# cchao0116/EasyDGL

Measured on AMD Instinct MI355X. Metric: sequences/sec (fwd+bwd+Adam) B=512 L=100 d=128 |I|=20K, higher is better.
Workload: dtype bf16

## Files before the change

easydgl_amd/csrc/k_tail.hip:

```cpp
#include "edgl_common.h"

#ifdef EDGL_PHASE_TIMING
__device__ unsigned long long g_phase_cycles[16];
#endif
#if defined(EDGL_PHASE_TIMING) && defined(EDGL_PHASE_BWD)
#define PHB_DECL PH_DECL
#define PHB_MARK(i) PH_MARK(i)
#define PHB_FLUSH() PH_FLUSH(0)
#else
#define PHB_DECL
#define PHB_MARK(i)
#define PHB_FLUSH()
#endif

namespace {

constexpr int MAXRT = 7;

struct TailP {
    const bf16* att; const bf16* xin; int ld_x;
    const bf16 *WoT, *WiT, *WoutT, *WtT;
    const float *bo, *bi, *bout, *bt, *g1, *b1, *g2, *b2, *g3, *b3;
    int B, T, C;
    float rate; const uint64_t* rng; uint32_t sid1, sid2;
    const int64_t* mpos; int M; int head; const int32_t* hmap;
    bf16 *ao, *a1, *pre_f, *f, *o, *y, *pre_t, *so, *hrows;
    float *st1, *st2, *st3;
    int dhp, dht;
};

template <int CT>
struct TailGeom {
    static constexpr int C = 16 * CT, NW = CT, NTHR = 64 * CT, LD = C + 8, CV = C / 8;
    static constexpr int LDF = C + 4;
    static constexpr size_t BUF = (size_t)MAXRT * 16 * LD * sizeof(bf16);
    static_assert((size_t)MAXRT * 16 * LDF * sizeof(float) <= 2 * BUF, "f32 staging image exceeds two buffers");
    static constexpr size_t SMEM = 4 * BUF + 64 * sizeof(float);
    static constexpr size_t SMEM_BWD = SMEM + (size_t)(MAXRT * 16 + 512) * sizeof(int);
    static constexpr int PAR_BO = 0, PAR_BOUT = 1, PAR_G1 = 2, PAR_B1 = 3, PAR_G2 = 4, PAR_B2 = 5, PAR_G3 = 6, PAR_B3 = 7, PAR_BT = 8, PAR_BI = 9;
    static constexpr size_t SMEM_FWD = SMEM + (size_t)11 * C * sizeof(float);
};

template <int CT>
struct RowImage {
    using G = TailGeom<CT>;
    static constexpr int NV = MAXRT * 16 * G::CV, NI = (NV + G::NTHR - 1) / G::NTHR;
    static_assert(NI * G::NTHR - NV < G::NTHR && NV >= G::NTHR, "last round: at most one repeat per thread");
    uint4 d[NI];
    static __device__ __forceinline__ int vec(int i) {
        const int v = threadIdx.x + i * G::NTHR;
        return v < NV ? v : v - (NI * G::NTHR - NV);
    }
    __device__ __forceinline__ void load(const bf16* src, long ld, int T) {
// ... 332 lines not shown
    {
        float mean, rstd;
        joint_moments<CT>(z, nrt, T, lane, red, mean, rstd, cpad);
        if (threadIdx.x == 0) { p.st3[2 * b] = mean; p.st3[2 * b + 1] = rstd; }
        const float4 v_g = *reinterpret_cast<const float4*>(par + G::PAR_G3 * C + nl), v_b = *reinterpret_cast<const float4*>(par + G::PAR_B3 * C + nl);
        const float gv[4] = {v_g.x, v_g.y, v_g.z, v_g.w}, ev[4] = {v_b.x, v_b.y, v_b.z, v_b.w};
#pragma unroll
        for (int rt = 0; rt < MAXRT; ++rt)
            if (rt < nrt) {
                float v[4];
#pragma unroll
                for (int r = 0; r < 4; ++r) v[r] = (z[rt][r] - mean) * rstd * gv[r] + ev[r];
                st_bf4(bufB + (rt * 16 + l15) * LD + nl, v);
            }
    }
    lds_barrier();
    if ((int)threadIdx.x < p.M * G::CV && gat_dst >= 0)
        *reinterpret_cast<uint4*>(p.hrows + gat_dst * C + (threadIdx.x % G::CV) * 8) =
            *reinterpret_cast<const uint4*>(bufB + gat_t * LD + (threadIdx.x % G::CV) * 8);
    for (int v = threadIdx.x + G::NTHR; v < p.M * G::CV; v += G::NTHR) {
        const int j = v / G::CV, cv = v % G::CV;
        const long src = (long)b * p.M + j;
        const int t = (int)p.mpos[src];
        const long dst = p.hmap ? (long)p.hmap[src] : src;
        if (dst >= 0) *reinterpret_cast<uint4*>(p.hrows + dst * C + cv * 8) = *reinterpret_cast<const uint4*>(bufB + t * LD + cv * 8);
    }
#if defined(EDGL_PHASE_TIMING) && !defined(EDGL_PHASE_BWD)
    PH_MARK(0);
    if ((threadIdx.x & 63) == 0) atomicAdd(&g_phase_cycles[8], ph_acc[0]);
#endif
}

struct TailBwdP {
    const bf16 *xin; int ld_x;
    const bf16 *ao, *a1, *pre_f, *o, *pre_t, *so;
    const float *st1, *st2, *st3;
    const bf16 *Wo, *Wi, *Wout, *Wt;
    const float *g1, *g2, *g3;
    int B, T, C;
    float rate; const uint64_t* rng; uint32_t sid1, sid2;
    int head;
    const bf16* d_rows; const int64_t* mpos; int M; const int32_t* rowmap;
    const bf16* d_y_in;
    bf16 *d_pre_t, *d_o, *d_pre_f, *d_ao, *d_res1, *d_att;
    float *part1, *part2, *part3;
    int dhp, dht;
};

template <int CT, int NKB>
__device__ __forceinline__ void tile_dx(const WFrags<NKB>& wf, const bf16* Gs, int nrt, int lane, f32x4 (&acc)[MAXRT]) {
    tile_gemm<CT, NKB>(wf, Gs, nrt, lane, acc);
}

template <int CT>
__device__ __forceinline__ void ln_bwd_regs(const float (&z)[MAXRT][4], const float (&dy)[MAXRT][4], float mean, float rstd,
                                            const float (&gv)[4], int nrt, int T, int lane, int nl, float* red, float* part_b,
                                            float (&dz)[MAXRT][4], const ChanPad& cp) {
    const int l15 = lane & 15;
    const float n = (float)T * cp.ctrue;
    float s1 = 0.f, s2 = 0.f, dga[4] = {0.f, 0.f, 0.f, 0.f}, dbe[4] = {0.f, 0.f, 0.f, 0.f};
#pragma unroll
    for (int rt = 0; rt < MAXRT; ++rt)
        if (rt < nrt && rt * 16 + l15 < T) {
#pragma unroll
            for (int r = 0; r < 4; ++r) {
                const float xh = (z[rt][r] - mean) * rstd, gg = dy[rt][r] * gv[r];
                s1 += gg; s2 += gg * xh; dga[r] += dy[rt][r] * xh; dbe[r] += dy[rt][r];
            }
        }
    const float m1 = block_sum_lds(s1, red) / n;
    const float m2 = block_sum_lds(s2, red) / n;
#pragma unroll
    for (int r = 0; r < 4; ++r) {
#pragma unroll
        for (int o = 1; o < 16; o <<= 1) { dga[r] += __shfl_xor(dga[r], o, 64); dbe[r] += __shfl_xor(dbe[r], o, 64); }
    }
    if (l15 == 0) {
#pragma unroll
        for (int r = 0; r < 4; ++r) { part_b[nl + r] = dbe[r]; part_b[16 * CT + nl + r] = dga[r]; }
    }
#pragma unroll
    for (int rt = 0; rt < MAXRT; ++rt)
#pragma unroll
        for (int r = 0; r < 4; ++r) {
            const float xh = (z[rt][r] - mean) * rstd;
            dz[rt][r] = cp.rm[r] * (rstd * (dy[rt][r] * gv[r] - m1 - xh * m2));
        }
}

template <int CT, int NRT>
__global__ __launch_bounds__(64 * CT) void tail_bwd_kernel(TailBwdP p) {
    using G = TailGeom<CT>;
    constexpr int C = G::C, LD = G::LD, NKB = C / 32;
    extern __shared__ __attribute__((aligned(16))) char smem[];
    bf16* bufA = reinterpret_cast<bf16*>(smem);
    bf16* bufS = reinterpret_cast<bf16*>(smem + G::BUF);
    bf16* bufB = reinterpret_cast<bf16*>(smem + 2 * G::BUF);
    bf16* bufC = reinterpret_cast<bf16*>(smem + 3 * G::BUF);
    float* red = reinterpret_cast<float*>(smem + 4 * G::BUF);
    int* rowmap = reinterpret_cast<int*>(red + 64);
    int* nextj = rowmap + MAXRT * 16;
    int* mpos_s = nextj + 256;
    const int b = blockIdx.x, T = p.T, nrt = NRT ? NRT : (T + 15) / 16;
    const int lane = threadIdx.x & 63, wave = threadIdx.x >> 6, g4 = (lane >> 4) * 4, l15 = lane & 15;
    const int n0 = wave * 16, nl = n0 + g4;
    const long row0 = (long)b * T;
    const ChanPad cpad = chan_pad<CT>(nl, p.dhp, p.dht);
    float z[MAXRT][4], dy[MAXRT][4], dz[MAXRT][4];
    WFrags<NKB> wf = p.head ? load_wfrags<NKB>(p.Wt + (long)n0 * C, C, lane) : load_wfrags<NKB>(p.Wout + (long)n0 * C, C, lane);
    PHB_DECL
    RowImage<CT> im_o, im_a;

    if (p.head) {
        const bool staged = p.M <= MAXRT * 16;
        constexpr int NG = RowImage<CT>::NI;
        int gsrc[NG];
        if (staged && p.rowmap) {
#pragma unroll
            for (int i = 0; i < NG; ++i) gsrc[i] = p.rowmap[(long)b * p.M + min(RowImage<CT>::vec(i) / G::CV, p.M - 1)];
        } else {
#pragma unroll
            for (int i = 0; i < NG; ++i) gsrc[i] = b * p.M + min(RowImage<CT>::vec(i) / G::CV, p.M - 1);
        }
        const int my_pos = (int)p.mpos[(long)b * p.M + min((int)threadIdx.x, p.M - 1)];
        RowImage<CT> im_so, im_dg;
        im_so.load(p.so + row0 * C, C, T);
        im_dg.load(p.pre_t + row0 * C, C, T);
        if (staged) {
            uint4 g[NG];
#pragma unroll
            for (int i = 0; i < NG; ++i)
                g[i] = *reinterpret_cast<const uint4*>(p.d_rows + (long)max(gsrc[i], 0) * C + (RowImage<CT>::vec(i) % G::CV) * 8);
            im_so.store(bufB, T);
            im_dg.store(bufA, T);
#pragma unroll
            for (int i = 0; i < NG; ++i) {
                const int v = RowImage<CT>::vec(i), j = v / G::CV, cv = v % G::CV;
                if (j < p.M) *reinterpret_cast<uint4*>(bufC + j * LD + cv * 8) = gsrc[i] >= 0 ? g[i] : make_uint4(0, 0, 0, 0);
            }
        } else {
// ... 199 lines not shown
#pragma unroll
    for (int rt = 0; rt < MAXRT; ++rt)
        if (rt < nrt) {
            const int row = rt * 16 + l15;
            float v[4], w[4];
#pragma unroll
            for (int r = 0; r < 4; ++r) {
                w[r] = dz[rt][r];
                v[r] = dz[rt][r];
            }
            drop_apply4(dk1, (uint64_t)((row0 + min(row, T - 1)) * C + nl), v);
            st_bf4(bufC + row * LD + nl, v);
            st_bf4(bufS + row * LD + nl, w);
        }
    lds_barrier();
    copy_out<CT>(p.d_ao + row0 * C, C, bufC, T);
    copy_out<CT>(p.d_res1 + row0 * C, C, bufS, T);
    PHB_MARK(6);
    {
        f32x4 acc[MAXRT];
#pragma unroll
        for (int rt = 0; rt < MAXRT; ++rt) acc[rt] = f32x4{0.f, 0.f, 0.f, 0.f};
        tile_dx<CT, NKB>(wf, bufC, nrt, lane, acc);
#pragma unroll
        for (int rt = 0; rt < MAXRT; ++rt)
            if (rt < nrt) {
                const float v[4] = {acc[rt][0], acc[rt][1], acc[rt][2], acc[rt][3]};
                st_bf4(bufA + (rt * 16 + l15) * LD + nl, v);
            }
    }
    lds_barrier();
    copy_out<CT>(p.d_att + row0 * C, C, bufA, T);
    PHB_MARK(7);
    PHB_FLUSH();
}

namespace t2 {
constexpr int C = 128, NTHR = 512, NKB = 4, TMAX = 101;
constexpr int IMG = TMAX * 256;
constexpr int OFF_RED = 3 * IMG, OFF_PAR = OFF_RED + 256;
constexpr int PAR_BOUT = 0, PAR_G2 = 1, PAR_B2 = 2, PAR_G3 = 3, PAR_B3 = 4, PAR_BI = 5, PAR_BT = 7, NPAR = 8;
constexpr int SMEM_FWD = OFF_PAR + NPAR * C * 4;
static_assert(SMEM_FWD == 81920, "two workgroups per CU");
constexpr int OFF_ROWMAP = OFF_RED + 256, OFF_NEXTJ = OFF_ROWMAP + MAXRT * 16 * 4, OFF_MPOS = OFF_NEXTJ + 256 * 4;
constexpr int SMEM_BWD = OFF_MPOS + 256 * 4;
static_assert(SMEM_BWD <= 81920, "two workgroups per CU");

struct Lane {
    int lane, wave, q, l15, nl;
    int frag[NKB];
    int quad;
    int squad;
};
__device__ __forceinline__ Lane make_lane() {
    Lane L;
    L.lane = threadIdx.x & 63; L.wave = threadIdx.x >> 6; L.q = L.lane >> 4; L.l15 = L.lane & 15; L.nl = L.wave * 16 + L.q * 4;
#pragma unroll
    for (int kb = 0; kb < NKB; ++kb) L.frag[kb] = L.l15 * 256 + (((kb * 4 + L.q) ^ L.l15) << 4);
    L.quad = L.l15 * 256 + (((L.wave * 2 + (L.q >> 1)) ^ L.l15) << 4) + ((L.q & 1) << 3);
    L.squad = L.l15 * 512 + (((L.wave * 4 + L.q) ^ L.l15) << 4);
    return L;
}
__device__ __forceinline__ int vec_off(int row, int cv) { return row * 256 + ((cv ^ (row & 15)) << 4); }

template <int NRT>
__device__ __forceinline__ void gemm(const WFrags<NKB>& wf, const char* img, const Lane& L, f32x4 (&acc)[MAXRT]) {
#pragma unroll
    for (int rt = 0; rt < NRT; ++rt) {
#pragma unroll
        for (int kb = 0; kb < NKB; ++kb)
            acc[rt] = mma_kblock(wf.w[kb], *reinterpret_cast<const Vec16<bf16>*>(img + L.frag[kb] + rt * 4096), acc[rt]);
        __builtin_amdgcn_sched_barrier(0);
    }
}
template <int NRT>
__device__ __forceinline__ void zero_acc(f32x4 (&acc)[MAXRT]) {
#pragma unroll
    for (int rt = 0; rt < MAXRT; ++rt) acc[rt] = f32x4{0.f, 0.f, 0.f, 0.f};
}
__device__ __forceinline__ void copy_in2(char* d0, const bf16* s0, long ld0, char* d1, const bf16* s1, long ld1, int T) {
    uint4 a[4], b[4];
    const int nv = T * 16;
#pragma unroll
    for (int i = 0; i < 4; ++i) {
        const int v = min((int)threadIdx.x + i * NTHR, nv - 1), row = v >> 4, cv = v & 15;
        a[i] = *reinterpret_cast<const uint4*>(s0 + (long)row * ld0 + cv * 8);
        b[i] = *reinterpret_cast<const uint4*>(s1 + (long)row * ld1 + cv * 8);
    }
#pragma unroll
    for (int i = 0; i < 4; ++i) {
        const int v = min((int)threadIdx.x + i * NTHR, nv - 1), row = v >> 4, cv = v & 15;
        *reinterpret_cast<uint4*>(d0 + vec_off(row, cv)) = a[i];
        *reinterpret_cast<uint4*>(d1 + vec_off(row, cv)) = b[i];
    }
}
__device__ __forceinline__ void copy_out(bf16* dst, long ld, const char* img, int T) {
    const int nv = T * 16;
#pragma unroll
    for (int i = 0; i < 4; ++i) {
        const int v = threadIdx.x + i * NTHR, row = v >> 4, cv = v & 15;
        if (v < nv) *reinterpret_cast<uint4*>(dst + (long)row * ld + cv * 8) = *reinterpret_cast<const uint4*>(img + vec_off(row, cv));
    }
}
template <int NRT>
__device__ __forceinline__ void stage_acc(char* stg, const f32x4 (&acc)[MAXRT], const Lane& L, int T) {
#pragma unroll
    for (int rt = 0; rt < NRT; ++rt)
        if (rt * 16 + L.l15 < T)
            *reinterpret_cast<float4*>(stg + L.squad + rt * 8192) = make_float4(acc[rt][0], acc[rt][1], acc[rt][2], acc[rt][3]);
}
template <bool SYNC>
__device__ __forceinline__ void gelu_pass(const char* stg, const float* bias_g, bf16* dact_g, bf16* act_g, long ldg, char* act_img, int T) {
    const int cv = threadIdx.x & 15, rsub = threadIdx.x >> 4;
    const float4 b0 = *reinterpret_cast<const float4*>(bias_g + cv * 8), b1 = *reinterpret_cast<const float4*>(bias_g + cv * 8 + 4);
    const int s0 = rsub * 512 + (((2 * cv) ^ (rsub & 15)) << 4);
// ... 148 lines not shown
    if (p.head) touch_regs(wf);
    copy_out(p.o + row0 * C, C, Q, T);
    {
        float mean, rstd;
        joint_moments<8>(z, NRT, T, L.lane, red, mean, rstd, cpad);
        if (threadIdx.x == 0) { p.st2[2 * b] = mean; p.st2[2 * b + 1] = rstd; }
        const float4 v_g = *reinterpret_cast<const float4*>(par + PAR_G2 * C + nl), v_b = *reinterpret_cast<const float4*>(par + PAR_B2 * C + nl);
        const float gv[4] = {v_g.x, v_g.y, v_g.z, v_g.w}, ev[4] = {v_b.x, v_b.y, v_b.z, v_b.w};
#pragma unroll
        for (int rt = 0; rt < NRT; ++rt) {
            float v[4];
#pragma unroll
            for (int r = 0; r < 4; ++r) v[r] = (z[rt][r] - mean) * rstd * gv[r] + ev[r];
            if (rt * 16 + l15 < T) st_bf4(reinterpret_cast<bf16*>(R + L.quad + rt * 4096), v);
        }
    }
    lds_barrier();
    copy_out(p.y + row0 * C, C, R, T);
    if (!p.head) return;
    zero_acc<NRT>(acc);
    gemm<NRT>(wf, R, L, acc);
    stage_acc<NRT>(P, acc, L, T);
    lds_barrier();
    gelu_pass<false>(P, par + PAR_BT * C, p.pre_t + row0 * C, p.so + row0 * C, C, R, T);
    lds_barrier();
#pragma unroll
    for (int rt = 0; rt < NRT; ++rt) ld_bf4(reinterpret_cast<const bf16*>(R + L.quad + rt * 4096), z[rt]);
    {
        float mean, rstd;
        joint_moments<8>(z, NRT, T, L.lane, red, mean, rstd, cpad);
        if (threadIdx.x == 0) { p.st3[2 * b] = mean; p.st3[2 * b + 1] = rstd; }
        const float4 v_g = *reinterpret_cast<const float4*>(par + PAR_G3 * C + nl), v_b = *reinterpret_cast<const float4*>(par + PAR_B3 * C + nl);
        const float gv[4] = {v_g.x, v_g.y, v_g.z, v_g.w}, ev[4] = {v_b.x, v_b.y, v_b.z, v_b.w};
#pragma unroll
        for (int rt = 0; rt < NRT; ++rt) {
            float v[4];
#pragma unroll
            for (int r = 0; r < 4; ++r) v[r] = (z[rt][r] - mean) * rstd * gv[r] + ev[r];
            if (rt * 16 + l15 < T) st_bf4(reinterpret_cast<bf16*>(Q + L.quad + rt * 4096), v);
        }
    }
    lds_barrier();
    if ((int)threadIdx.x < p.M * 16 && gat_dst >= 0)
        *reinterpret_cast<uint4*>(p.hrows + gat_dst * C + (threadIdx.x & 15) * 8) = *reinterpret_cast<const uint4*>(Q + vec_off(gat_t, threadIdx.x & 15));
    for (int v = threadIdx.x + NTHR; v < p.M * 16; v += NTHR) {
        const int j = v >> 4, cv = v & 15;
        const long src = (long)b * p.M + j;
        const int t = (int)p.mpos[src];
        const long dst = p.hmap ? (long)p.hmap[src] : src;
        if (dst >= 0) *reinterpret_cast<uint4*>(p.hrows + dst * C + cv * 8) = *reinterpret_cast<const uint4*>(Q + vec_off(t, cv));
    }
}

}

__global__ void tail_pack_kernel(const bf16* Wo, const bf16* Wi, const bf16* Wout, const bf16* Wt, int C, bf16* pack) {
    const long cc = (long)C * C;
    for (long i = (long)blockIdx.x * blockDim.x + threadIdx.x; i < 6 * cc; i += (long)gridDim.x * blockDim.x) {
        const bf16* src; long off; int K, N;
        if (i < cc) { src = Wo; off = 0; K = C; N = C; }
        else if (i < 3 * cc) { src = Wi; off = cc; K = C; N = 2 * C; }
        else if (i < 5 * cc) { src = Wout; off = 3 * cc; K = 2 * C; N = C; }
        else { src = Wt; off = 5 * cc; K = C; N = C; }
        const long j = i - off;
        const int n = (int)(j / K), k = (int)(j % K);
        pack[i] = src[(long)k * N + n];
    }
}

}

static int g_tail2 = -1;
static bool tail2_enabled() {
    if (g_tail2 < 0) g_tail2 = edgl_env_on("EDGL_TAIL2") ? 1 : 0;
    return g_tail2 != 0;
}
extern "C" int edgl_tail_variant(int variant) {
    const int prev = tail2_enabled() ? 1 : 0;
    if (variant >= 0) g_tail2 = variant ? 1 : 0;
    return prev;
}

extern "C" long edgl_tail_pack_elems(int C) { return 6L * C * C; }

extern "C" int edgl_tail_supported(int T, int C, int dtype) { return dtype == EDGL_BF16 && (C == 64 || C == 128) && T >= 1 && T <= 16 * MAXRT; }

extern "C" int edgl_tail_pack(const void* Wo, const void* Wi, const void* Wout, const void* Wt, int C, void* pack, void* stream) {
    EDGL_REQUIRE(Wo && Wi && Wout && Wt && pack, EDGL_ERR_NULL, "edgl_tail_pack: null pointer");
    EDGL_REQUIRE(C == 64 || C == 128, EDGL_ERR_SHAPE, "edgl_tail_pack: C=%d unsupported (64 or 128)", C);
    hipLaunchKernelGGL(tail_pack_kernel, dim3(96), dim3(256), 0, (hipStream_t)stream, (const bf16*)Wo, (const bf16*)Wi,
                       (const bf16*)Wout, (const bf16*)Wt, C, (bf16*)pack);
    EDGL_LAUNCH_CHECK();
    return EDGL_OK;
}

extern "C" int edgl_tail_fwd_ct(const void* att, const void* xin, int ld_x, const void* pack, const float* bo, const float* bi,
                             const float* bout, const float* bt, const float* g1, const float* b1, const float* g2,
                             const float* b2, const float* g3, const float* b3, int B, int T, int C, float drop_rate,
                             const uint64_t* rng_state, uint32_t sid1, uint32_t sid2, const int64_t* masked_pos, int M, int head,
                             void* ao, void* a1, float* st1, void* pre_f, void* f, void* o, void* y, float* st2, void* pre_t,
                             void* so, float* st3, void* hrows, const int32_t* hrow_map, int dh_pad, int dh_true, int dtype,
                                void* stream) {
    EDGL_REQUIRE(att && xin && pack && bo && bi && bout && g1 && b1 && g2 && b2 && ao && a1 && st1 && pre_f && f && o && y && st2,
                 EDGL_ERR_NULL, "edgl_tail_fwd: null pointer");
    EDGL_REQUIRE(!head || (bt && g3 && b3 && masked_pos && pre_t && so && st3 && hrows && M >= 1), EDGL_ERR_NULL,
                 "edgl_tail_fwd: the head needs its weights, positions and outputs");
    EDGL_REQUIRE(B > 0 && edgl_tail_supported(T, C, dtype) && ld_x % 8 == 0, EDGL_ERR_SHAPE,
                 "edgl_tail_fwd: unsupported shape B=%d T=%d C=%d dtype=%d (bf16, C in {64,128}, T <= 112)", B, T, C, dtype);
    EDGL_REQUIRE(drop_rate == 0.f || rng_state, EDGL_ERR_NULL, "edgl_tail_fwd: dropout without rng_state");
    EDGL_REQUIRE((dh_pad == 0 && dh_true == 0) || (dh_pad > 0 && (dh_pad & (dh_pad - 1)) == 0 && dh_true > 0 && dh_true <= dh_pad && C % dh_pad == 0),
                 EDGL_ERR_SHAPE, "edgl_tail_fwd: padded-channel spec dh_pad=%d dh_true=%d does not fit C=%d", dh_pad, dh_true, C);
    const bf16* pk = (const bf16*)pack;
    const long cc = (long)C * C;
    TailP p{(const bf16*)att, (const bf16*)xin, ld_x, pk, pk + cc, pk + 3 * cc, pk + 5 * cc, bo, bi, bout, bt, g1, b1, g2, b2, g3, b3,
            B, T, C, drop_rate, rng_state, sid1, sid2, masked_pos, M, head, hrow_map, (bf16*)ao, (bf16*)a1, (bf16*)pre_f, (bf16*)f, (bf16*)o,
            (bf16*)y, (bf16*)pre_t, (bf16*)so, (bf16*)hrows, st1, st2, st3, dh_pad, dh_true};
    hipStream_t st = (hipStream_t)stream;
    const int nrt = (T + 15) / 16;
    if (tail2_enabled() && C == 128 && T <= t2::TMAX) {
        auto k2 = nrt <= 2 ? t2::tail2_fwd_kernel<2> : nrt <= 4 ? t2::tail2_fwd_kernel<4> : t2::tail2_fwd_kernel<MAXRT>;
        hipFuncSetAttribute((const void*)k2, hipFuncAttributeMaxDynamicSharedMemorySize, t2::SMEM_FWD);
        hipLaunchKernelGGL(k2, dim3(B), dim3(t2::NTHR), t2::SMEM_FWD, st, p);
        EDGL_LAUNCH_CHECK();
        return EDGL_OK;
    }
    auto k = C == 128 ? (nrt <= 2 ? tail_fwd_kernel<8, 2> : nrt <= 4 ? tail_fwd_kernel<8, 4> : tail_fwd_kernel<8, MAXRT>)
                      : (nrt <= 2 ? tail_fwd_kernel<4, 2> : nrt <= 4 ? tail_fwd_kernel<4, 4> : tail_fwd_kernel<4, MAXRT>);
    const size_t smem = C == 128 ? TailGeom<8>::SMEM_FWD : TailGeom<4>::SMEM_FWD;
    hipFuncSetAttribute((const void*)k, hipFuncAttributeMaxDynamicSharedMemorySize, (int)smem);
    hipLaunchKernelGGL(k, dim3(B), dim3(C == 128 ? 512 : 256), smem, st, p);
    EDGL_LAUNCH_CHECK();
    return EDGL_OK;
}

extern "C" int edgl_tail_fwd(const void* att, const void* xin, int ld_x, const void* pack, const float* bo, const float* bi,
                             const float* bout, const float* bt, const float* g1, const float* b1, const float* g2,
                             const float* b2, const float* g3, const float* b3, int B, int T, int C, float drop_rate,
                             const uint64_t* rng_state, uint32_t sid1, uint32_t sid2, const int64_t* masked_pos, int M, int head,
                             void* ao, void* a1, float* st1, void* pre_f, void* f, void* o, void* y, float* st2, void* pre_t,
                             void* so, float* st3, void* hrows, const int32_t* hrow_map, int dtype, void* stream) {
    return edgl_tail_fwd_ct(att, xin, ld_x, pack, bo, bi, bout, bt, g1, b1, g2, b2, g3, b3, B, T, C, drop_rate, rng_state, sid1, sid2,
                            masked_pos, M, head, ao, a1, st1, pre_f, f, o, y, st2, pre_t, so, st3, hrows, hrow_map, 0, 0, dtype, stream);
}
extern "C" int edgl_tail_bwd_ct(const void* xin, int ld_x, const void* ao, const void* a1, const void* pre_f, const void* o,
                             const void* pre_t, const void* so, const float* st1, const float* st2, const float* st3,
                             const void* Wo, const void* Wi, const void* Wout, const void* Wt, const float* g1, const float* g2,
                             const float* g3, int B, int T, int C, float drop_rate, const uint64_t* rng_state, uint32_t sid1,
                             uint32_t sid2, int head, const void* d_rows, const int64_t* masked_pos, int M,
                             const int32_t* dy_rowmap, const void* d_y_in, void* d_pre_t, void* d_o, void* d_pre_f, void* d_ao,
                             void* d_res1, void* d_att, float* dg1, float* db1, float* dg2, float* db2, float* dg3, float* db3,
                             float* workspace, int dh_pad, int dh_true, int dtype, void* stream) {
    EDGL_REQUIRE(xin && ao && a1 && pre_f && o && st1 && st2 && Wo && Wi && Wout && g1 && g2 && d_o && d_pre_f && d_ao && d_res1 &&
                 d_att && dg1 && db1 && dg2 && db2 && workspace, EDGL_ERR_NULL, "edgl_tail_bwd: null pointer");
    EDGL_REQUIRE(head ? (pre_t && so && st3 && Wt && g3 && d_rows && masked_pos && d_pre_t && dg3 && db3 && M >= 1 && M <= 256) : (d_y_in != nullptr),
                 EDGL_ERR_NULL, "edgl_tail_bwd: head needs its tensors (M <= 256); without it d_y_in is the upstream gradient");
    EDGL_REQUIRE(B > 0 && edgl_tail_supported(T, C, dtype) && ld_x % 8 == 0, EDGL_ERR_SHAPE,
                 "edgl_tail_bwd: unsupported shape B=%d T=%d C=%d dtype=%d", B, T, C, dtype);
    EDGL_REQUIRE(drop_rate == 0.f || rng_state, EDGL_ERR_NULL, "edgl_tail_bwd: dropout without rng_state");
    EDGL_REQUIRE((dh_pad == 0 && dh_true == 0) || (dh_pad > 0 && (dh_pad & (dh_pad - 1)) == 0 && dh_true > 0 && dh_true <= dh_pad && C % dh_pad == 0),
                 EDGL_ERR_SHAPE, "edgl_tail_bwd: padded-channel spec dh_pad=%d dh_true=%d does not fit C=%d", dh_pad, dh_true, C);
    float* part1 = workspace; float* part2 = workspace + (long)B * 2 * C; float* part3 = workspace + (long)B * 4 * C;
    TailBwdP p{(const bf16*)xin, ld_x, (const bf16*)ao, (const bf16*)a1, (const bf16*)pre_f, (const bf16*)o, (const bf16*)pre_t,
               (const bf16*)so, st1, st2, st3, (const bf16*)Wo, (const bf16*)Wi, (const bf16*)Wout, (const bf16*)Wt, g1, g2, g3, B, T, C,
               drop_rate, rng_state, sid1, sid2, head, (const bf16*)d_rows, masked_pos, M, dy_rowmap, (const bf16*)d_y_in,
               (bf16*)d_pre_t, (bf16*)d_o, (bf16*)d_pre_f, (bf16*)d_ao, (bf16*)d_res1, (bf16*)d_att, part1, part2, part3, dh_pad, dh_true};
    hipStream_t st = (hipStream_t)stream;
    const int nrt = (T + 15) / 16;
    auto k = C == 128 ? (nrt <= 2 ? tail_bwd_kernel<8, 2> : nrt <= 4 ? tail_bwd_kernel<8, 4> : tail_bwd_kernel<8, MAXRT>)
                      : (nrt <= 2 ? tail_bwd_kernel<4, 2> : nrt <= 4 ? tail_bwd_kernel<4, 4> : tail_bwd_kernel<4, MAXRT>);
    const size_t smem = C == 128 ? TailGeom<8>::SMEM_BWD : TailGeom<4>::SMEM_BWD;
    hipFuncSetAttribute((const void*)k, hipFuncAttributeMaxDynamicSharedMemorySize, (int)smem);
    hipLaunchKernelGGL(k, dim3(B), dim3(C == 128 ? 512 : 256), smem, st, p);
    EDGL_LAUNCH_CHECK();
    auto red2 = [&](float* part, float* dg, float* db) -> int {
        if (dg == db + C) return edgl_reduce_rows(part, B, 2 * C, 2L * C, db, 0, st);
        int rc = edgl_reduce_rows(part, B, C, 2L * C, db, 0, st);
        if (rc) return rc;
        return edgl_reduce_rows(part + C, B, C, 2L * C, dg, 0, st);
    };
    int rc = red2(part1, dg1, db1);
    if (rc) return rc;
    rc = red2(part2, dg2, db2);
    if (rc) return rc;
    if (head) rc = red2(part3, dg3, db3);
    return rc;
}
extern "C" int edgl_tail_bwd(const void* xin, int ld_x, const void* ao, const void* a1, const void* pre_f, const void* o,
                             const void* pre_t, const void* so, const float* st1, const float* st2, const float* st3,
                             const void* Wo, const void* Wi, const void* Wout, const void* Wt, const float* g1, const float* g2,
                             const float* g3, int B, int T, int C, float drop_rate, const uint64_t* rng_state, uint32_t sid1,
                             uint32_t sid2, int head, const void* d_rows, const int64_t* masked_pos, int M,
                             const int32_t* dy_rowmap, const void* d_y_in, void* d_pre_t, void* d_o, void* d_pre_f, void* d_ao,
                             void* d_res1, void* d_att, float* dg1, float* db1, float* dg2, float* db2, float* dg3, float* db3,
                             float* workspace, int dtype, void* stream) {
    return edgl_tail_bwd_ct(xin, ld_x, ao, a1, pre_f, o, pre_t, so, st1, st2, st3, Wo, Wi, Wout, Wt, g1, g2, g3, B, T, C, drop_rate, rng_state,
                            sid1, sid2, head, d_rows, masked_pos, M, dy_rowmap, d_y_in, d_pre_t, d_o, d_pre_f, d_ao, d_res1, d_att, dg1, db1,
                            dg2, db2, dg3, db3, workspace, 0, 0, dtype, stream);
}

extern "C" long edgl_tail_bwd_workspace(int B, int C) { return 6L * B * C; }

#ifdef EDGL_PHASE_TIMING
extern "C" int edgl_debug_phase_cycles_tail(unsigned long long* out16, int reset) {
    if (hipMemcpyFromSymbol(out16, HIP_SYMBOL(g_phase_cycles), 16 * sizeof(unsigned long long)) != hipSuccess) return -1;
    if (reset) {
        unsigned long long z[16] = {0};
        if (hipMemcpyToSymbol(HIP_SYMBOL(g_phase_cycles), z, sizeof(z)) != hipSuccess) return -1;
    }
    return 0;
}
#endif
```

Baseline: 689,000.

## Add two-per-CU tail backward kernel with register-resident quads and cached LDS attributes

Adds a new tail2 backward kernel for C=128 that fits in 80 KB of LDS so two workgroups can share a CU. It keeps operand quads in registers and prefetches the next stage's inputs and weights during the GEMMs. It also stores gamma tables in LDS and overlaps the output copies with later phases. The hipFuncSetAttribute calls move into a per-device call_once so they are no longer paid on every launch. The cost is a large new code path with tighter register pressure, and a dependency on the tail2 toggle being enabled by default.

```diff
diff --git a/easydgl_amd/csrc/k_tail.hip b/easydgl_amd/csrc/k_tail.hip
--- a/easydgl_amd/csrc/k_tail.hip
+++ b/easydgl_amd/csrc/k_tail.hip
@@ -1,4 +1,5 @@
 #include "edgl_common.h"
+#include <mutex>
 
 #ifdef EDGL_PHASE_TIMING
 __device__ unsigned long long g_phase_cycles[16];
@@ -437,40 +438,50 @@
     tile_gemm<CT, NKB>(wf, Gs, nrt, lane, acc);
 }
 
+template <int CT, bool STORE>
+__device__ __forceinline__ void ln_bwd_part(const float (&z)[MAXRT][4], const float (&dy)[MAXRT][4], float mean, float rstd,
+                                            const float (&gv)[4], int nrt, int T, int lane, int nl, float* red, float* part_b,
+                                            float (&dz)[MAXRT][4], const ChanPad& cp, float (&dga)[4], float (&dbe)[4]) {
+    const int l15 = lane & 15;
+    const float n = (float)T * cp.ctrue;
+    float s1 = 0.f, s2 = 0.f;
+#pragma unroll
+    for (int r = 0; r < 4; ++r) dga[r] = dbe[r] = 0.f;
+#pragma unroll
+    for (int rt = 0; rt < MAXRT; ++rt)
+        if (rt < nrt && rt * 16 + l15 < T) {
+#pragma unroll
+            for (int r = 0; r < 4; ++r) {
+                const float xh = (z[rt][r] - mean) * rstd, gg = dy[rt][r] * gv[r];
+                s1 += gg; s2 += gg * xh; dga[r] += dy[rt][r] * xh; dbe[r] += dy[rt][r];
+            }
+        }
+    const float m1 = block_sum_lds(s1, red) / n;
+    const float m2 = block_sum_lds(s2, red) / n;
+#pragma unroll
+    for (int r = 0; r < 4; ++r) {
+#pragma unroll
+        for (int o = 1; o < 16; o <<= 1) { dga[r] += __shfl_xor(dga[r], o, 64); dbe[r] += __shfl_xor(dbe[r], o, 64); }
+    }
+    if (STORE && l15 == 0) {
+#pragma unroll
+        for (int r = 0; r < 4; ++r) { part_b[nl + r] = dbe[r]; part_b[16 * CT + nl + r] = dga[r]; }
+    }
+#pragma unroll
+    for (int rt = 0; rt < MAXRT; ++rt)
+#pragma unroll
+        for (int r = 0; r < 4; ++r) {
+            const float xh = (z[rt][r] - mean) * rstd;
+            dz[rt][r] = cp.rm[r] * (rstd * (dy[rt][r] * gv[r] - m1 - xh * m2));
+            if (!STORE && r == 3) __builtin_amdgcn_sched_barrier(0);
+        }
+}
 template <int CT>
 __device__ __forceinline__ void ln_bwd_regs(const float (&z)[MAXRT][4], const float (&dy)[MAXRT][4], float mean, float rstd,
                                             const float (&gv)[4], int nrt, int T, int lane, int nl, float* red, float* part_b,
                                             float (&dz)[MAXRT][4], const ChanPad& cp) {
-    const int l15 = lane & 15;
-    const float n = (float)T * cp.ctrue;
-    float s1 = 0.f, s2 = 0.f, dga[4] = {0.f, 0.f, 0.f, 0.f}, dbe[4] = {0.f, 0.f, 0.f, 0.f};
-#pragma unroll
-    for (int rt = 0; rt < MAXRT; ++rt)
-        if (rt < nrt && rt * 16 + l15 < T) {
-#pragma unroll
-            for (int r = 0; r < 4; ++r) {
-                const float xh = (z[rt][r] - mean) * rstd, gg = dy[rt][r] * gv[r];
-                s1 += gg; s2 += gg * xh; dga[r] += dy[rt][r] * xh; dbe[r] += dy[rt][r];
-            }
-        }
-    const float m1 = block_sum_lds(s1, red) / n;
-    const float m2 = block_sum_lds(s2, red) / n;
-#pragma unroll
-    for (int r = 0; r < 4; ++r) {
-#pragma unroll
-        for (int o = 1; o < 16; o <<= 1) { dga[r] += __shfl_xor(dga[r], o, 64); dbe[r] += __shfl_xor(dbe[r], o, 64); }
-    }
-    if (l15 == 0) {
-#pragma unroll
-        for (int r = 0; r < 4; ++r) { part_b[nl + r] = dbe[r]; part_b[16 * CT + nl + r] = dga[r]; }
-    }
-#pragma unroll
-    for (int rt = 0; rt < MAXRT; ++rt)
-#pragma unroll
-        for (int r = 0; r < 4; ++r) {
-            const float xh = (z[rt][r] - mean) * rstd;
-            dz[rt][r] = cp.rm[r] * (rstd * (dy[rt][r] * gv[r] - m1 - xh * m2));
-        }
+    float dga[4], dbe[4];
+    ln_bwd_part<CT, true>(z, dy, mean, rstd, gv, nrt, T, lane, nl, red, part_b, dz, cp, dga, dbe);
 }
 
 template <int CT, int NRT>
@@ -776,15 +787,22 @@
     int quad;
     int squad;
 };
-__device__ __forceinline__ Lane make_lane() {
+__device__ __forceinline__ Lane make_lane(int tid) {
     Lane L;
-    L.lane = threadIdx.x & 63; L.wave = threadIdx.x >> 6; L.q = L.lane >> 4; L.l15 = L.lane & 15; L.nl = L.wave * 16 + L.q * 4;
+    L.lane = tid & 63; L.wave = tid >> 6; L.q = L.lane >> 4; L.l15 = L.lane & 15; L.nl = L.wave * 16 + L.q * 4;
 #pragma unroll
     for (int kb = 0; kb < NKB; ++kb) L.frag[kb] = L.l15 * 256 + (((kb * 4 + L.q) ^ L.l15) << 4);
     L.quad = L.l15 * 256 + (((L.wave * 2 + (L.q >> 1)) ^ L.l15) << 4) + ((L.q & 1) << 3);
     L.squad = L.l15 * 512 + (((L.wave * 4 + L.q) ^ L.l15) << 4);
     return L;
 }
+__device__ __forceinline__ Lane make_lane() { return make_lane(threadIdx.x); }
+__device__ __forceinline__ int fresh_tid() {
+    int t = threadIdx.x;
+    asm volatile("" : "+v"(t));
+    return t;
+}
+__device__ __forceinline__ Lane fresh_lane() { return make_lane(fresh_tid()); }
 __device__ __forceinline__ int vec_off(int row, int cv) { return row * 256 + ((cv ^ (row & 15)) << 4); }
 
 template <int NRT>
@@ -1039,6 +1057,318 @@
     }
 }
 
+struct Quads { uint2 q[MAXRT]; };
+template <int NRT>
+__device__ __forceinline__ Quads load_quads(const bf16* src, int ld, int T) {
+    Quads a;
+    const Lane L = fresh_lane();
+#pragma unroll
+    for (int rt = 0; rt < NRT; ++rt)
+        a.q[rt] = *reinterpret_cast<const uint2*>(reinterpret_cast<const char*>(src) + (uint32_t)((min(rt * 16 + L.l15, T - 1) * ld + L.nl) * 2));
+#pragma unroll
+    for (int rt = NRT; rt < MAXRT; ++rt) a.q[rt] = make_uint2(0u, 0u);
+    return a;
+}
+__device__ __forceinline__ void quad_f32(const uint2& q, float (&v)[4]) {
+    Frag4<bf16> f;
+    *reinterpret_cast<uint2*>(&f) = q;
+#pragma unroll
+    for (int r = 0; r < 4; ++r) v[r] = to_f32(f.v[r]);
+}
+__device__ __forceinline__ int quad_off(int row, const Lane& L) {
+    return row * 256 + (((L.wave * 2 + (L.q >> 1)) ^ (row & 15)) << 4) + ((L.q & 1) << 3);
+}
+__device__ __forceinline__ void store_part(float* part_b, const Lane& L, const float (&dga)[4], const float (&dbe)[4]) {
+    if (L.l15 == 0) {
+#pragma unroll
+        for (int r = 0; r < 4; ++r) { part_b[L.nl + r] = dbe[r]; part_b[C + L.nl + r] = dga[r]; }
+    }
+}
+
+__device__ __forceinline__ void copy_out_b(bf16* dst, int ld, const char* img, int T) {
+    const int nv = T * 16, tid = fresh_tid();
+#pragma unroll
+    for (int i = 0; i < 4; ++i) {
+        const int v = tid + i * NTHR, row = v >> 4, cv = v & 15;
+        if (v < nv) *reinterpret_cast<uint4*>(reinterpret_cast<char*>(dst) + (uint32_t)((row * ld + cv * 8) * 2)) = *reinterpret_cast<const uint4*>(img + vec_off(row, cv));
+    }
+}
+
+constexpr int OFF_GAM = SMEM_BWD, SMEM_BWD_ALL = 81920;
+static_assert(OFF_GAM + 3 * C * 4 <= SMEM_BWD_ALL, "gamma table");
+static_assert(2 * IMG + MAXRT * 4096 <= SMEM_BWD_ALL && 2 * IMG + MAXRT * 4096 <= SMEM_FWD, "operand reads of rows >= T leave the workgroup's LDS");
+
+template <int NRT>
+__global__ __launch_bounds__(NTHR, 4) void tail2_bwd_kernel(TailBwdP p) {
+    extern __shared__ __attribute__((aligned(16))) char smem[];
+    char* const P = smem; char* const Q = smem + IMG; char* const R = smem + 2 * IMG;
+    float* red = reinterpret_cast<float*>(smem + OFF_RED);
+    int* rowmap = reinterpret_cast<int*>(smem + OFF_ROWMAP);
+    int* nextj = reinterpret_cast<int*>(smem + OFF_NEXTJ);
+    int* mpos_s = reinterpret_cast<int*>(smem + OFF_MPOS);
+    float* gam = reinterpret_cast<float*>(smem + OFF_GAM);
+    const int b = blockIdx.x, T = p.T;
+    const Lane L = make_lane();
+    const int n0 = L.wave * 16, nl = L.nl, l15 = L.l15;
+    const long row0 = (long)b * T;
+    auto make_cpad = [&]() { int n = nl; asm volatile("" : "+v"(n)); return chan_pad<8>(n, p.dhp, p.dht); };
+    const uint64_t idx0 = (uint64_t)((row0 + l15) * C + nl);
+    PHB_DECL
+    if ((int)threadIdx.x < C) {
+        const int c = threadIdx.x;
+        const float* g3_or = p.head ? p.g3 : p.g1;
+        const float x0 = p.g1[c], x1 = p.g2[c], x2 = g3_or[c];
+        gam[c] = x0; gam[C + c] = x1; gam[2 * C + c] = x2;
+    }
+    DropKey dk1 = make_dropkey(p.rng, p.sid1, p.rate), dk2 = make_dropkey(p.rng, p.sid2, p.rate);
+    dk1.scale = __uint_as_float(__builtin_amdgcn_readfirstlane(__float_as_uint(dk1.scale)));
+    dk2.scale = __uint_as_float(__builtin_amdgcn_readfirstlane(__float_as_uint(dk2.scale)));
+    auto uni = [](float v) { return __uint_as_float(__builtin_amdgcn_readfirstlane(__float_as_uint(v))); };
+    const float* st3_or = p.head ? p.st3 : p.st1;
+    const float mean1 = uni(p.st1[2 * b]), rstd1 = uni(p.st1[2 * b + 1]), mean2 = uni(p.st2[2 * b]), rstd2 = uni(p.st2[2 * b + 1]),
+                mean3 = uni(st3_or[2 * b]), rstd3 = uni(st3_or[2 * b + 1]);
+    float z[MAXRT][4], dy[MAXRT][4], dz[MAXRT][4], dga[4], dbe[4];
+    f32x4 acc[MAXRT];
+    WFrags<NKB> wf;
+    Quads qa, qb;
+
+    if (p.head) {
+        int gsrc[4];
+        if (p.rowmap) {
+#pragma unroll
+            for (int i = 0; i < 4; ++i) gsrc[i] = p.rowmap[(long)b * p.M + min((int)(threadIdx.x + i * NTHR) >> 4, p.M - 1)];
+        } else {
+#pragma unroll
+            for (int i = 0; i < 4; ++i) gsrc[i] = b * p.M + min((int)(threadIdx.x + i * NTHR) >> 4, p.M - 1);
+        }
+        const int my_pos = (int)p.mpos[(long)b * p.M + min((int)threadIdx.x, p.M - 1)];
+        qa = load_quads<NRT>(p.so + row0 * C, C, T);
+        qb = load_quads<NRT>(p.pre_t + row0 * C, C, T);
+        {
+            uint4 g[4];
+#pragma unroll
+            for (int i = 0; i < 4; ++i) g[i] = *reinterpret_cast<const uint4*>(p.d_rows + (long)max(gsrc[i], 0) * C + (threadIdx.x & 15) * 8);
+#pragma unroll
+            for (int i = 0; i < 4; ++i) {
+                const int j = (int)(threadIdx.x + i * NTHR) >> 4;
+                if (j < p.M) *reinterpret_cast<uint4*>(P + vec_off(j, threadIdx.x & 15)) = gsrc[i] >= 0 ? g[i] : make_uint4(0, 0, 0, 0);
+            }
+        }
+        if ((int)threadIdx.x < p.M) mpos_s[threadIdx.x] = my_pos;
+        if ((int)threadIdx.x < MAXRT * 16) rowmap[threadIdx.x] = -1;
+        lds_barrier();
+        if ((int)threadIdx.x < p.M) {
+            const int j = threadIdx.x, t = mpos_s[j];
+            int nxt = -1;
+            bool first = true;
+#pragma unroll 8
+            for (int k = 0; k < p.M; ++k) {
+                const bool same = mpos_s[k] == t;
+                nxt = (same && k > j && nxt < 0) ? k : nxt;
+                first = first && !(same && k < j);
+            }
+            nextj[j] = nxt;
+            if (first) rowmap[t] = j;
+        }
+        lds_barrier();
+        int jn[MAXRT];
+        {
+            int jh[MAXRT];
+#pragma unroll
+            for (int rt = 0; rt < NRT; ++rt) {
+                const int row = rt * 16 + l15;
+                quad_f32(qa.q[rt], z[rt]);
+                jh[rt] = row < T ? rowmap[row] : -1;
+                __builtin_amdgcn_sched_barrier(0);
+            }
+#pragma unroll
+            for (int rt = 0; rt < NRT; ++rt) {
+                jn[rt] = nextj[max(jh[rt], 0)];
+                ld_bf4(reinterpret_cast<const bf16*>(P + quad_off(max(jh[rt], 0), L)), dy[rt]);
+#pragma unroll
+                for (int r = 0; r < 4; ++r) dy[rt][r] = jh[rt] >= 0 ? dy[rt][r] : 0.f;
+                jn[rt] = jh[rt] >= 0 ? jn[rt] : -1;
+                __builtin_amdgcn_sched_barrier(0);
+            }
+        }
+#pragma unroll
+        for (int rt = 0; rt < NRT; ++rt)
+            for (int j = jn[rt]; j >= 0; j = nextj[j]) {
+                float v[4];
+                ld_bf4(reinterpret_cast<const bf16*>(P + quad_off(j, L)), v);
+#pragma unroll
+                for (int r = 0; r < 4; ++r) dy[rt][r] += v[r];
+            }
+        PHB_MARK(0);
+        {
+            const float4 gg = *reinterpret_cast<const float4*>(gam + 2 * C + nl);
+            const float gv[4] = {gg.x, gg.y, gg.z, gg.w};
+            ln_bwd_part<8, false>(z, dy, mean3, rstd3, gv, NRT, T, L.lane, nl, red, nullptr, dz, make_cpad(), dga, dbe);
+        }
+#pragma unroll
+        for (int rt = 0; rt < NRT; ++rt) {
+            float dg[4];
+            quad_f32(qb.q[rt], dg);
+            const float v[4] = {dz[rt][0] * dg[0], dz[rt][1] * dg[1], dz[rt][2] * dg[2], dz[rt][3] * dg[3]};
+            if (rt * 16 + l15 < T) st_bf4(reinterpret_cast<bf16*>(R + L.quad + rt * 4096), v);
+            __builtin_amdgcn_sched_barrier(0);
+        }
+        lds_barrier();
+        store_part(p.part3 + (long)b * 2 * C, L, dga, dbe);
+        copy_out_b(p.d_pre_t + row0 * C, C, R, T);
+        EDGL_PIN();
+        wf = load_wfrags<NKB>(p.Wt + (long)n0 * C, C, L.lane);
+        qa = load_quads<NRT>(p.o + row0 * C, C, T);
+        qb = load_quads<NRT>(p.a1 + row0 * C, C, T);
+        zero_acc<NRT>(acc);
+        gemm<NRT>(wf, R, fresh_lane(), acc);
+#pragma unroll
+        for (int rt = 0; rt < NRT; ++rt)
+#pragma unroll
+            for (int r = 0; r < 4; ++r) dy[rt][r] = rbf(acc[rt][r]);
+        PHB_MARK(1);
+    } else {
+        qa = load_quads<NRT>(p.d_y_in + row0 * C, C, T);
+#pragma unroll
+        for (int rt = 0; rt < NRT; ++rt) quad_f32(qa.q[rt], dy[rt]);
+        qa = load_quads<NRT>(p.o + row0 * C, C, T);
+        qb = load_quads<NRT>(p.a1 + row0 * C, C, T);
+        lds_barrier();
+        touch_regs(qa); touch_regs(qb);
+    }
+#pragma unroll
+    for (int rt = 0; rt < NRT; ++rt) {
+        float ov[4], av[4];
+        quad_f32(qa.q[rt], ov);
+        quad_f32(qb.q[rt], av);
+        drop_apply4(dk2, idx0 + (uint64_t)(rt * 16 * C), ov);
+#pragma unroll
+        for (int r = 0; r < 4; ++r) z[rt][r] = ov[r] + av[r];
+        __builtin_amdgcn_sched_barrier(0);
+    }
+    PHB_MARK(2);
+    {
+        const float4 gg = *reinterpret_cast<const float4*>(gam + C + nl);
+        const float gv[4] = {gg.x, gg.y, gg.z, gg.w};
+        ln_bwd_part<8, false>(z, dy, mean2, rstd2, gv, NRT, T, L.lane, nl, red, nullptr, dz, make_cpad(), dga, dbe);
+    }
+#pragma unroll
+    for (int rt = 0; rt < NRT; ++rt) {
+        float v[4], w[4];
+#pragma unroll
+        for (int r = 0; r < 4; ++r) {
+            w[r] = rbf(dz[rt][r]);
+            v[r] = dz[rt][r];
+        }
+        drop_apply4(dk2, idx0 + (uint64_t)(rt * 16 * C), v);
+        if (rt * 16 + l15 < T) {
+            st_bf4(reinterpret_cast<bf16*>(P + L.quad + rt * 4096), w);
+            st_bf4(reinterpret_cast<bf16*>(Q + L.quad + rt * 4096), v);
+        }
+        __builtin_amdgcn_sched_barrier(0);
+    }
+    lds_barrier();
+    store_part(p.part2 + (long)b * 2 * C, L, dga, dbe);
+    copy_out_b(p.d_o + row0 * C, C, Q, T);
+    EDGL_PIN();
+    qa = load_quads<NRT>(p.pre_f + row0 * 2 * C, 2 * C, T);
+    wf = load_wfrags<NKB>(p.Wout + (long)n0 * C, C, L.lane);
+    WFrags<NKB> wi = load_wfrags<NKB>(p.Wi + (long)n0 * 2 * C, 2 * C, L.lane);
+    PHB_MARK(3);
+    f32x4 acc6[MAXRT];
+    zero_acc<NRT>(acc6);
+#pragma unroll
+    for (int h = 0; h < 2; ++h) {
+        const Lane F = fresh_lane();
+#pragma unroll
+        for (int rt = 0; rt < NRT; ++rt) {
+            f32x4 a = f32x4{0.f, 0.f, 0.f, 0.f};
+#pragma unroll
+            for (int kb = 0; kb < NKB; ++kb) a = mma_kblock(wf.w[kb], *reinterpret_cast<const Vec16<bf16>*>(Q + F.frag[kb] + rt * 4096), a);
+            float dg[4];
+            quad_f32(qa.q[rt], dg);
+            const float v[4] = {a[0] * dg[0], a[1] * dg[1], a[2] * dg[2], a[3] * dg[3]};
+            if (rt * 16 + l15 < T) st_bf4(reinterpret_cast<bf16*>(R + L.quad + rt * 4096), v);
+            if (rt & 1) __builtin_amdgcn_sched_barrier(0);
+        }
+        if (h == 1) {
+            EDGL_PIN();
+            wi = load_wfrags<NKB>(p.Wi + (long)n0 * 2 * C + C, 2 * C, L.lane);
+        }
+        lds_barrier();
+        copy_out_b(p.d_pre_f + row0 * 2 * C + h * C, 2 * C, R, T);
+        EDGL_PIN();
+        if (h == 0) {
+            qa = load_quads<NRT>(p.pre_f + row0 * 2 * C + C, 2 * C, T);
+            wf = load_wfrags<NKB>(p.Wout + (long)(C + n0) * C, C, L.lane);
+        } else {
+            qa = load_quads<NRT>(p.ao + row0 * C, C, T);
+            qb = load_quads<NRT>(p.xin + row0 * p.ld_x, p.ld_x, T);
+        }
+        gemm<NRT>(wi, R, fresh_lane(), acc6);
+        lds_barrier();
+    }
+#pragma unroll
+    for (int rt = 0; rt < NRT; ++rt) {
+        float da[4];
+        ld_bf4(reinterpret_cast<const bf16*>(P + L.quad + rt * 4096), da);
+#pragma unroll
+        for (int r = 0; r < 4; ++r) dy[rt][r] = rbf(acc6[rt][r] + da[r]);
+        __builtin_amdgcn_sched_barrier(0);
+    }
+    PHB_MARK(4);
+#pragma unroll
+    for (int rt = 0; rt < NRT; ++rt) {
+        float ov[4], xv[4];
+        quad_f32(qa.q[rt], ov);
+        quad_f32(qb.q[rt], xv);
+        drop_apply4(dk1, idx0 + (uint64_t)(rt * 16 * C), ov);
+#pragma unroll
+        for (int r = 0; r < 4; ++r) z[rt][r] = ov[r] + xv[r];
+        __builtin_amdgcn_sched_barrier(0);
+    }
+    PHB_MARK(5);
+    {
+        const float4 gg = *reinterpret_cast<const float4*>(gam + nl);
+        const float gv[4] = {gg.x, gg.y, gg.z, gg.w};
+        ln_bwd_part<8, false>(z, dy, mean1, rstd1, gv, NRT, T, L.lane, nl, red, nullptr, dz, make_cpad(), dga, dbe);
+    }
+#pragma unroll
+    for (int rt = 0; rt < NRT; ++rt) {
+        float v[4], w[4];
+#pragma unroll
+        for (int r = 0; r < 4; ++r) {
+            w[r] = dz[rt][r];
+            v[r] = dz[rt][r];
+        }
+        drop_apply4(dk1, idx0 + (uint64_t)(rt * 16 * C), v);
+        if (rt * 16 + l15 < T) {
+            st_bf4(reinterpret_cast<bf16*>(Q + L.quad + rt * 4096), v);
+            st_bf4(reinterpret_cast<bf16*>(R + L.quad + rt * 4096), w);
+        }
+        __builtin_amdgcn_sched_barrier(0);
+    }
+    lds_barrier();
+    store_part(p.part1 + (long)b * 2 * C, L, dga, dbe);
+    copy_out_b(p.d_ao + row0 * C, C, Q, T);
+    copy_out_b(p.d_res1 + row0 * C, C, R, T);
+    EDGL_PIN();
+    wf = load_wfrags<NKB>(p.Wo + (long)n0 * C, C, L.lane);
+    PHB_MARK(6);
+    zero_acc<NRT>(acc);
+    gemm<NRT>(wf, Q, fresh_lane(), acc);
+#pragma unroll
+    for (int rt = 0; rt < NRT; ++rt) {
+        const float v[4] = {acc[rt][0], acc[rt][1], acc[rt][2], acc[rt][3]};
+        if (rt * 16 + l15 < T) st_bf4(reinterpret_cast<bf16*>(P + L.quad + rt * 4096), v);
+        __builtin_amdgcn_sched_barrier(0);
+    }
+    lds_barrier();
+    copy_out_b(p.d_att + row0 * C, C, P, T);
+    PHB_MARK(7);
+    PHB_FLUSH();
+}
+
 }
 
 __global__ void tail_pack_kernel(const bf16* Wo, const bf16* Wi, const bf16* Wout, const bf16* Wt, int C, bf16* pack) {
@@ -1066,6 +1396,32 @@
     const int prev = tail2_enabled() ? 1 : 0;
     if (variant >= 0) g_tail2 = variant ? 1 : 0;
     return prev;
+}
+
+static bool tail_lds_attrs() {
+    constexpr int MAXDEV = 64;
+    static std::once_flag once[MAXDEV];
+    static bool ok[MAXDEV] = {};
+    int dev = 0;
+    if (hipGetDevice(&dev) != hipSuccess || dev < 0 || dev >= MAXDEV) return false;
+    std::call_once(once[dev], [dev] {
+        bool good = true;
+        auto set = [&](const void* f, size_t bytes) { good = hipFuncSetAttribute(f, hipFuncAttributeMaxDynamicSharedMemorySize, (int)bytes) == hipSuccess && good; };
+        set((const void*)tail_fwd_kernel<8, 2>, TailGeom<8>::SMEM_FWD); set((const void*)tail_fwd_kernel<8, 4>, TailGeom<8>::SMEM_FWD);
+        set((const void*)tail_fwd_kernel<8, MAXRT>, TailGeom<8>::SMEM_FWD);
+        set((const void*)tail_fwd_kernel<4, 2>, TailGeom<4>::SMEM_FWD); set((const void*)tail_fwd_kernel<4, 4>, TailGeom<4>::SMEM_FWD);
+        set((const void*)tail_fwd_kernel<4, MAXRT>, TailGeom<4>::SMEM_FWD);
+        set((const void*)tail_bwd_kernel<8, 2>, TailGeom<8>::SMEM_BWD); set((const void*)tail_bwd_kernel<8, 4>, TailGeom<8>::SMEM_BWD);
+        set((const void*)tail_bwd_kernel<8, MAXRT>, TailGeom<8>::SMEM_BWD);
+        set((const void*)tail_bwd_kernel<4, 2>, TailGeom<4>::SMEM_BWD); set((const void*)tail_bwd_kernel<4, 4>, TailGeom<4>::SMEM_BWD);
+        set((const void*)tail_bwd_kernel<4, MAXRT>, TailGeom<4>::SMEM_BWD);
+        set((const void*)t2::tail2_fwd_kernel<2>, t2::SMEM_FWD); set((const void*)t2::tail2_fwd_kernel<4>, t2::SMEM_FWD);
+        set((const void*)t2::tail2_fwd_kernel<MAXRT>, t2::SMEM_FWD);
+        set((const void*)t2::tail2_bwd_kernel<2>, t2::SMEM_BWD_ALL); set((const void*)t2::tail2_bwd_kernel<4>, t2::SMEM_BWD_ALL);
+        set((const void*)t2::tail2_bwd_kernel<MAXRT>, t2::SMEM_BWD_ALL);
+        ok[dev] = good;
+    });
+    return ok[dev];
 }
 
 extern "C" long edgl_tail_pack_elems(int C) { return 6L * C * C; }
@@ -1106,7 +1462,7 @@
     const int nrt = (T + 15) / 16;
     if (tail2_enabled() && C == 128 && T <= t2::TMAX) {
         auto k2 = nrt <= 2 ? t2::tail2_fwd_kernel<2> : nrt <= 4 ? t2::tail2_fwd_kernel<4> : t2::tail2_fwd_kernel<MAXRT>;
-        hipFuncSetAttribute((const void*)k2, hipFuncAttributeMaxDynamicSharedMemorySize, t2::SMEM_FWD);
+        EDGL_REQUIRE(tail_lds_attrs(), EDGL_ERR_LAUNCH, "edgl_tail_fwd (two per CU): hipFuncSetAttribute failed on this device");
         hipLaunchKernelGGL(k2, dim3(B), dim3(t2::NTHR), t2::SMEM_FWD, st, p);
         EDGL_LAUNCH_CHECK();
         return EDGL_OK;
@@ -1114,7 +1470,7 @@
     auto k = C == 128 ? (nrt <= 2 ? tail_fwd_kernel<8, 2> : nrt <= 4 ? tail_fwd_kernel<8, 4> : tail_fwd_kernel<8, MAXRT>)
                       : (nrt <= 2 ? tail_fwd_kernel<4, 2> : nrt <= 4 ? tail_fwd_kernel<4, 4> : tail_fwd_kernel<4, MAXRT>);
     const size_t smem = C == 128 ? TailGeom<8>::SMEM_FWD : TailGeom<4>::SMEM_FWD;
-    hipFuncSetAttribute((const void*)k, hipFuncAttributeMaxDynamicSharedMemorySize, (int)smem);
+    EDGL_REQUIRE(tail_lds_attrs(), EDGL_ERR_LAUNCH, "edgl_tail_fwd (one per CU): hipFuncSetAttribute failed on this device");
     hipLaunchKernelGGL(k, dim3(B), dim3(C == 128 ? 512 : 256), smem, st, p);
     EDGL_LAUNCH_CHECK();
     return EDGL_OK;
@@ -1153,11 +1509,16 @@
                (bf16*)d_pre_t, (bf16*)d_o, (bf16*)d_pre_f, (bf16*)d_ao, (bf16*)d_res1, (bf16*)d_att, part1, part2, part3, dh_pad, dh_true};
     hipStream_t st = (hipStream_t)stream;
     const int nrt = (T + 15) / 16;
-    auto k = C == 128 ? (nrt <= 2 ? tail_bwd_kernel<8, 2> : nrt <= 4 ? tail_bwd_kernel<8, 4> : tail_bwd_kernel<8, MAXRT>)
-                      : (nrt <= 2 ? tail_bwd_kernel<4, 2> : nrt <= 4 ? tail_bwd_kernel<4, 4> : tail_bwd_kernel<4, MAXRT>);
-    const size_t smem = C == 128 ? TailGeom<8>::SMEM_BWD : TailGeom<4>::SMEM_BWD;
-    hipFuncSetAttribute((const void*)k, hipFuncAttributeMaxDynamicSharedMemorySize, (int)smem);
-    hipLaunchKernelGGL(k, dim3(B), dim3(C == 128 ? 512 : 256), smem, st, p);
+    EDGL_REQUIRE(tail_lds_attrs(), EDGL_ERR_LAUNCH, "edgl_tail_bwd: hipFuncSetAttribute failed on this device");
+    if (tail2_enabled() && C == 128 && T <= t2::TMAX && (!head || M <= MAXRT * 16)) {
+        auto k2 = nrt <= 2 ? t2::tail2_bwd_kernel<2> : nrt <= 4 ? t2::tail2_bwd_kernel<4> : t2::tail2_bwd_kernel<MAXRT>;
+        hipLaunchKernelGGL(k2, dim3(B), dim3(t2::NTHR), t2::SMEM_BWD_ALL, st, p);
+    } else {
+        auto k = C == 128 ? (nrt <= 2 ? tail_bwd_kernel<8, 2> : nrt <= 4 ? tail_bwd_kernel<8, 4> : tail_bwd_kernel<8, MAXRT>)
+                          : (nrt <= 2 ? tail_bwd_kernel<4, 2> : nrt <= 4 ? tail_bwd_kernel<4, 4> : tail_bwd_kernel<4, MAXRT>);
+        const size_t smem = C == 128 ? TailGeom<8>::SMEM_BWD : TailGeom<4>::SMEM_BWD;
+        hipLaunchKernelGGL(k, dim3(B), dim3(C == 128 ? 512 : 256), smem, st, p);
+    }
     EDGL_LAUNCH_CHECK();
     auto red2 = [&](float* part, float* dg, float* db) -> int {
         if (dg == db + C) return edgl_reduce_rows(part, B, 2 * C, 2L * C, db, 0, st);
```

New measurement: 706,900 (median of 6 runs). 2.6% higher.
